# mdejong/MetalHuffman

Hardware: AMD Instinct MI355X
Metric: decoded MB/s (and Mpixels/s) at 2048×1536 grayscale, 1/2/4/8 GPU + CPU ref (higher is better)
Workload: dtype u8; 1 GPU; config2: one 2048x1536 BigBridge-derived frame per launch per GPU; width=2048, height=1536, parallelism=frame-sharded x1

## Files before the change

### metalhuffman_amd/csrc/mh_decode.hip

```cpp
#include <hip/hip_runtime.h>
#include <hip/hip_ext.h>

#include <stdint.h>

#include <atomic>
#include <mutex>

#include "../../include/metalhuffman.h"
#include "mh_lut.hpp"

namespace {

#ifndef MH_DIAG_STAMPS
#define MH_DIAG_STAMPS 0
#endif
#ifndef MH_DIAG_CLOCK
#define MH_DIAG_CLOCK 0
#endif
#ifndef MH_DIAG_ARGS
#define MH_DIAG_ARGS 0
#endif
#ifndef MH_DIAG_DROP_STORES
#define MH_DIAG_DROP_STORES 0
#endif
#ifndef MH_LANE_PAIRS
#define MH_LANE_PAIRS 0
#endif
constexpr int kStageBytes = 4352;
constexpr int kMaxWavesPerWG = 8;
constexpr int kMinWavesPerEU = 6;
constexpr int kBatchStoreAux = 2;
constexpr int kSmallStoreAux = 18;
static_assert(kStageBytes % 16 == 0, "stage uses 16-byte chunks");

typedef unsigned int v4u32 __attribute__((ext_vector_type(4)));

struct DecodeArgs {
  const uint32_t *offsets;
  const uint8_t *codes;
  const uint64_t *frame_off;
  uint64_t codes_bytes;
  const uint16_t *t1;
  const uint16_t *t2;
  const uint16_t *lut;
  const uint8_t *block_init;
  uint8_t *out;
  uint64_t out_pitch;
  uint64_t out_frame_stride;
  uint64_t out_frame_bytes;
  uint32_t t2_entries;
  uint32_t w, h, bw, bh, nb;
  uint32_t tiles_per_frame, total_tiles;
  uint32_t n_groups;
  uint32_t nwaves, grid;
};

__device__ __forceinline__ uint32_t bswap32(uint32_t x) {
  return __builtin_amdgcn_perm(0u, x, 0x00010203u);
}

__device__ __forceinline__ uint32_t split_lookup(const uint16_t *t1, const uint16_t *t2,
                                                 uint32_t t2_entries, uint32_t pat16) {
  uint32_t e = t1[pat16 >> 8];
  if ((e >> 8) == 0) {
    const uint32_t idx = (e & 0xFFu) * 256u + (pat16 & 0xFFu);
    e = idx < t2_entries ? (uint32_t)t2[idx] : 0u;
  }
  return e;
}


template <class SyncFn>
__device__ void build_lut(const uint16_t *t1, const uint16_t *t2, uint32_t t2_entries,
                          uint16_t *lut, uint32_t *p0, uint32_t tid, uint32_t nthreads,
                          SyncFn sync) {
  if (tid == 0) *p0 = (uint32_t)kL1Entries;
  sync();
  for (uint32_t p = tid; p < (uint32_t)kL1Entries; p += nthreads) {
    const uint32_t e = split_lookup(t1, t2, t2_entries, p << kL2Bits);
    lut[p] = (uint16_t)step_word(e);
    if ((e >> 8) > (uint32_t)kLutBits) atomicMin(p0, p);
  }
  for (uint32_t i = tid; i < (uint32_t)(kLutEntries - kL1Entries); i += nthreads)
    lut[kL1Entries + i] = 0;
  sync();
  const uint32_t P0 = *p0;
  for (uint32_t p = P0 + tid; p < (uint32_t)kL1Entries; p += nthreads) {
    const uint32_t sub = p - P0 + 1;
    lut[p] = (uint16_t)(sub < (uint32_t)kL2Subtables ? sub : 0u);
  }
  const uint32_t nl2 = ((uint32_t)kL1Entries - P0) << kL2Bits;
  for (uint32_t i = tid; i < nl2 && i < (uint32_t)(kL2Entries - (1 << kL2Bits)); i += nthreads)
    lut[kL1Entries + (1 << kL2Bits) + i] =
        (uint16_t)step_word(split_lookup(t1, t2, t2_entries, (P0 << kL2Bits) + i));
  sync();
}


#if !MH_LANE_PAIRS
__global__ void __launch_bounds__(1024) mh_prepare_lut_kernel(const uint16_t *t1, const uint16_t *t2,
                                                              uint32_t t2_entries, uint8_t *buf) {
  __shared__ uint16_t s_t1[256];
  __shared__ uint32_t s_scratch[4];
  if (threadIdx.x < 256) s_t1[threadIdx.x] = t1[threadIdx.x];
  __syncthreads();
  build_prepared_lut(s_t1, t2, t2_entries, buf, s_scratch);
}
#endif

struct LdsWords {
  const uint8_t *w;
  __device__ __forceinline__ const uint8_t *at(uint32_t byte_off) const { return w + byte_off; }
};
__device__ __forceinline__ uint32_t swz_off(uint32_t o) { return o ^ ((o >> 3) & 0x70u); }

__device__ __forceinline__ uint32_t pack_prev4(uint32_t a, uint32_t b, uint32_t c, uint32_t d) {
  const uint32_t lo = __builtin_amdgcn_perm(b, a, 0x0C0C0501u);
  const uint32_t hi = __builtin_amdgcn_perm(d, c, 0x05010C0Cu);
  return lo | hi;
}

__device__ __forceinline__ uint32_t pack_lo4(uint32_t a, uint32_t b, uint32_t c, uint32_t d) {
  const uint32_t lo = __builtin_amdgcn_perm(b, a, 0x0C0C0400u);
  const uint32_t hi = __builtin_amdgcn_perm(d, c, 0x04000C0Cu);
  return lo | hi;
}

__device__ __forceinline__ constexpr uint32_t ins_sel1(int j) {
  return j == 0 ? 0x03020105u : j == 1 ? 0x03020500u : j == 2 ? 0x03050100u : 0x05020100u;
}

__shared__ __attribute__((aligned(16))) uint16_t s_lut[kLutEntries];
__shared__ __attribute__((aligned(16))) uint8_t s_stage[kMaxWavesPerWG * kStageBytes];
__shared__ uint32_t s_p0;

#if MH_DIAG_STAMPS
constexpr int kDiagWaves = 8192, kDiagSlots = 8;
__device__ unsigned long long g_stamps[kDiagWaves * kDiagSlots];
#define MH_STAMP(i) (ts[i] = __builtin_amdgcn_s_memrealtime())
#else
#define MH_STAMP(i) ((void)0)
#endif

__device__ __forceinline__ void set_prio(uint32_t p) {
  switch (__builtin_amdgcn_readfirstlane(p) & 3u) {
    case 0: __builtin_amdgcn_s_setprio(0); break;
    case 1: __builtin_amdgcn_s_setprio(1); break;
    case 2: __builtin_amdgcn_s_setprio(2); break;
    default: __builtin_amdgcn_s_setprio(3); break;
  }
}

template <int kBits, bool kMaskedRefill, bool kEscapes = kBits == kLutBits, bool kSwizzle = false,
          int kStoreAux = kBatchStoreAux, bool kLazyRefill = false, bool kFlat8Bytes = false>
struct StepCfg {
  static constexpr bool kLazy = kLazyRefill;
  static constexpr bool kFlat8 = kFlat8Bytes;
  static constexpr int kAux = kStoreAux;
  static constexpr bool kEsc = kEscapes;
  static constexpr bool kSwz = kSwizzle;
  static constexpr bool kMasked = kMaskedRefill;
  static constexpr uint32_t kCur = 127u - (uint32_t)kBits;
  static constexpr uint32_t kMask = (2u << kBits) - 2u;
  static constexpr uint32_t kRefillAt = kCur - 32u;
};

using Lut13 = StepCfg<kLutBits, true>;
using Lut13NoEsc = StepCfg<kLutBits, true, false>;
using Lut13Flat = StepCfg<kLutBits, true, false, true>;

template <bool kDelta, class Cfg, class Src>
__device__ __forceinline__ void decode_block(const Src &src, const uint8_t *lut, uint32_t p,
                                             uint32_t prev, __amdgpu_buffer_rsrc_t out,
                                             uint32_t row0, uint32_t pitch, bool dead) {
  if constexpr (Cfg::kFlat8) {
    typedef const __attribute__((address_space(3))) uint32_t *lds_u32;
    typedef unsigned int v2u32 __attribute__((ext_vector_type(2)));
    const lds_u32 wp = (lds_u32)(src.w + (p >> 5) * 4u);
    const uint32_t sh = p & 31u;
    uint32_t w[17];
#pragma unroll
    for (int j = 0; j < 17; ++j) w[j] = wp[j];
    const uint32_t rbase = dead ? 0x80000000u : row0;
    uint32_t s = prev;
#pragma unroll
    for (uint32_t r = 0; r < 8; ++r) {
      uint32_t c[2];
#pragma unroll
      for (int h = 0; h < 2; ++h) {
        const uint32_t j = 2 * r + h;
        c[h] = (uint32_t)(((((uint64_t)w[j]) << 32 | w[j + 1]) << sh) >> 32);
      }
      v2u32 v;
      if (kDelta) {
        uint32_t sv[4];
#pragma unroll
        for (int h = 0; h < 2; ++h) {
#pragma unroll
          for (int i = 0; i < 4; ++i) sv[i] = s = s + ((c[h] >> (24 - 8 * i)) & 0xFFu);
          const uint32_t o = pack_lo4(sv[0], sv[1], sv[2], sv[3]);
          if (h) v.y = o; else v.x = o;
        }
      } else {
        v.x = bswap32(c[0]);
        v.y = bswap32(c[1]);
      }
      __builtin_amdgcn_raw_buffer_store_b64(v, out, (int)(rbase + r * pitch), 0, Cfg::kAux);
    }
    return;
  }
  typedef const __attribute__((address_space(3))) uint8_t *lds_u8;
  typedef const __attribute__((address_space(3))) uint32_t *lds_u32;
  const lds_u8 base = (lds_u8)src.w;
  lds_u8 wa = base + (p >> 5) * 4u;
  const auto rd = [&](lds_u8 q) -> uint32_t {
    if constexpr (Cfg::kSwz)
      return *(lds_u32)(base + swz_off((uint32_t)(q - base)));
    else
      return *(lds_u32)q;
  };
  uint32_t S = (prev << 8) + Cfg::kCur - (p & 31u);
  uint32_t kRefill = Cfg::kRefillAt;
  if constexpr ((Cfg::kRefillAt & 1u) != 0u) asm("s_mov_b32 %0, %1" : "=s"(kRefill) : "n"(Cfg::kRefillAt));
  uint32_t hi = rd(wa);
  uint32_t lo = rd(wa + 4);
  uint32_t nw = rd(wa + 8);

#define MH_LOOKUP(A1)                                                               \
  uint32_t e = *reinterpret_cast<const uint16_t *>(lut + (A1));
#define MH_FINISH(J, OW)                                                            \
  {                                                                                 \
    if constexpr (Cfg::kEsc) {                                                      \
      const bool esc = e < kEscapeBelow;                                            \
      if (__builtin_expect(__ballot(esc) != 0, 0)) {                                \
        const uint64_t x = (((uint64_t)hi) << 32) | lo;                             \
        const uint32_t x3 = (uint32_t)(x >> ((S - 2u) & 63u)) & 7u;                 \
        const uint32_t e2 = *reinterpret_cast<const uint16_t *>(                    \
            lut + 2u * (kL1Entries + ((e & 0xFFu) << kL2Bits) + x3));               \
        e = esc ? e2 : e;                                                           \
      }                                                                             \
    }                                                                               \
    S += e;                                                                         \
    if (kDelta) {                                                                   \
      sv[J] = S;                           \
    } else {                                                                        \
      OW = __builtin_amdgcn_perm(e + 0xFFu, OW, ins_sel1(J));    \
    }                                                                               \
  }
#define MH_STEP(J, OW)                                                              \
  {                                                                                 \
    const uint64_t x = (((uint64_t)hi) << 32) | lo;                                 \
    MH_LOOKUP((uint32_t)(x >> (S & 63u)) & Cfg::kMask)                              \
    MH_FINISH(J, OW)                                                                \
  }
#define MH_REFILL_C(c)                                                              \
  {                                                                                 \
    hi = c ? lo : hi;                                                               \
    lo = c ? nw : lo;                                                               \
    const uint32_t d = c ? 4u : 0u;                                                 \
    wa += d;                                                                        \
      \
      \
    if constexpr (Cfg::kSwz) asm volatile("" : "+v"(wa));                          \
      \
      \
      \
    if constexpr (Cfg::kMasked) asm volatile("" : "+v"(hi), "+v"(lo));             \
    S += d * 8u;                                                                    \
    if constexpr (!Cfg::kMasked) nw = rd(wa + 8);                                   \
  }
#define MH_STEP_L(J, OW)                                                            \
  {                                                                                 \
    const uint64_t x = (((uint64_t)hi) << 32) | lo;                                 \
    MH_LOOKUP((uint32_t)(x >> (S & 63u)) & Cfg::kMask)                              \
                        \
    const bool c = (S & 0xFFu) <= kRefill;                                         \
    hi = c ? lo : hi;                                                               \
    lo = c ? nw : lo;                                                               \
    const uint32_t d = c ? 4u : 0u;                                                 \
    wa += d;                                                                        \
    S += d * 8u;                                                                    \
      \
      \
    asm volatile("" : "+v"(S), "+v"(hi), "+v"(lo));                                \
      \
     \
     \
    if constexpr (((J) & 1) == 0) nw = rd(wa + 8);                                 \
    MH_FINISH(J, OW)                                                                \
  }
#define MH_STEP_R(J, OW)                                                            \
  {                                                                                 \
    const bool c = (S & 0xFFu) <= kRefill;                                         \
    MH_REFILL_C(c)                                                                  \
    MH_STEP(J, OW)                                                                  \
     \
     \
    if constexpr (Cfg::kMasked) {                                                   \
      if (c) nw = rd(wa + 8);                                                       \
    }                                                                               \
  }

  const uint32_t rbase = (dead || MH_DIAG_DROP_STORES) ? 0x80000000u : row0;
#pragma unroll
  for (uint32_t r = 0; r < 8; ++r) {
    uint32_t o0 = 0, o1 = 0;
    uint32_t sv[4];
    (void)sv;
    if constexpr (Cfg::kLazy) {
      MH_STEP_L(0, o0);
      MH_STEP_L(1, o0);
      MH_STEP_L(2, o0);
      MH_STEP_L(3, o0);
      if (kDelta) o0 = pack_prev4(sv[0], sv[1], sv[2], sv[3]);
      MH_STEP_L(0, o1);
      MH_STEP_L(1, o1);
      MH_STEP_L(2, o1);
      MH_STEP_L(3, o1);
      if (kDelta) o1 = pack_prev4(sv[0], sv[1], sv[2], sv[3]);
    } else {
    if (r) {
      MH_STEP_R(0, o0);
    } else {
      MH_STEP(0, o0);
    }
    MH_STEP(1, o0);
    MH_STEP_R(2, o0);
    MH_STEP(3, o0);
    if (kDelta) o0 = pack_prev4(sv[0], sv[1], sv[2], sv[3]);
    MH_STEP_R(0, o1);
    MH_STEP(1, o1);
    MH_STEP_R(2, o1);
    MH_STEP(3, o1);
    if (kDelta) o1 = pack_prev4(sv[0], sv[1], sv[2], sv[3]);
    }
    {
      typedef unsigned int v2u32 __attribute__((ext_vector_type(2)));
      v2u32 v;
      v.x = o0;
      v.y = o1;
      const uint32_t off = rbase + r * pitch;
      __builtin_amdgcn_raw_buffer_store_b64(v, out, (int)off, 0, Cfg::kAux);
    }
  }
#undef MH_STEP
#undef MH_STEP_R
#undef MH_STEP_L
#undef MH_LOOKUP
#undef MH_FINISH
#undef MH_REFILL_C
}

constexpr int kStageChunks = (kStageBytes / 16 + 63) / 64;

__device__ __forceinline__ __amdgpu_buffer_rsrc_t uniform_rsrc(const void *base, uint32_t bytes) {
  const uint64_t p = (uint64_t)base;
  const uint32_t lo = __builtin_amdgcn_readfirstlane((uint32_t)p);
  const uint32_t hi = __builtin_amdgcn_readfirstlane((uint32_t)(p >> 32));
  return __builtin_amdgcn_make_buffer_rsrc((void *)(((uint64_t)hi << 32) | lo), (short)0,
                                           (int)__builtin_amdgcn_readfirstlane(bytes), 0x00020000);
}

__device__ __forceinline__ uint32_t frame_of(const DecodeArgs &a, uint32_t tile) {
  if (a.total_tiles <= a.tiles_per_frame) return 0u;
  return tile / a.tiles_per_frame;
}

struct TileHdr {
  uint32_t tile;
  uint32_t off;
  uint32_t nxt;
  uint32_t fo_lo, fo_hi;
  uint32_t init;
};

__device__ __forceinline__ void hdr_issue(const DecodeArgs &a, uint32_t tile, uint32_t lane,
                                          TileHdr &h) {
  tile = __builtin_amdgcn_readfirstlane(tile);
  const bool live = tile < a.total_tiles;
  const uint32_t f = live ? frame_of(a, tile) : 0u;
  const uint32_t b = (live ? (tile - f * a.tiles_per_frame) * 64u : 0u) + lane;
  h.tile = tile;
  const __amdgpu_buffer_rsrc_t ro = uniform_rsrc(a.offsets + (uint64_t)f * a.nb, live ? a.nb * 4u : 0u);
  h.off = __builtin_amdgcn_raw_buffer_load_b32(ro, (int)(b * 4u), 0, 0);
  h.nxt = __builtin_amdgcn_raw_buffer_load_b32(ro, (int)(b * 4u + 4u), 0, 0);
  typedef unsigned int v2u32 __attribute__((ext_vector_type(2)));
  const __amdgpu_buffer_rsrc_t rf = uniform_rsrc(
      a.frame_off ? (const void *)a.frame_off : (const void *)a.offsets,
      (live && a.frame_off) ? 0x7FFFFFF0u : 0u);
  const v2u32 v = __builtin_amdgcn_raw_buffer_load_b64(rf, (int)((f + (lane & 1u)) * 8u), 0, 0);
  h.fo_lo = v.x;
  h.fo_hi = v.y;
  const __amdgpu_buffer_rsrc_t ri = uniform_rsrc(
      a.block_init ? (const void *)(a.block_init + (uint64_t)f * a.nb) : (const void *)a.offsets,
      (live && a.block_init) ? a.nb : 0u);
  h.init = __builtin_amdgcn_raw_buffer_load_b8(ri, (int)b, 0, 0);
}

struct Tile {
  uint32_t tile, f, b0;
  bool valid;
  uint32_t p;
  uint32_t start;
  uint32_t span;
  uint32_t fb32;
  uint64_t fbeg;
  uint32_t init;
  uint32_t span_end_bits;
};

__device__ __forceinline__ Tile hdr_resolve(const DecodeArgs &a, const TileHdr &h, uint32_t lane) {
  Tile t;
  t.tile = h.tile;
  t.f = frame_of(a, h.tile);
  t.b0 = (h.tile - t.f * a.tiles_per_frame) * 64u;
  const uint32_t b = t.b0 + lane;
  t.valid = b < a.nb;
  uint64_t fbytes = a.codes_bytes;
  t.fbeg = 0;
  if (a.frame_off) {
    const uint64_t lo = ((uint64_t)__builtin_amdgcn_readlane(h.fo_hi, 0) << 32) |
                        __builtin_amdgcn_readlane(h.fo_lo, 0);
    const uint64_t hi = ((uint64_t)__builtin_amdgcn_readlane(h.fo_hi, 1) << 32) |
                        __builtin_amdgcn_readlane(h.fo_lo, 1);
    t.fbeg = lo;
    fbytes = hi - lo;
  }
  t.fb32 = (uint32_t)(fbytes > 0xFFFFFFF0ull ? 0xFFFFFFF0ull : fbytes);
  const uint32_t fbits = t.fb32 > 0x1FFFFFFFu ? 0xFFFFFFFFu : t.fb32 * 8u;
  const uint32_t end_l = (b + 1u < a.nb) ? h.nxt : min(fbits, h.off + 64u * 16u);
  const uint32_t last = min(63u, a.nb - 1u - t.b0);
  const uint32_t sb = __builtin_amdgcn_readfirstlane(h.off);
  const uint32_t eb = __builtin_amdgcn_readlane(end_l, last);
  t.span_end_bits = eb;
  t.start = (sb >> 3) & ~15u;
  uint32_t end = (eb >> 3) + 24u;
  if (end > t.fb32 + 16u) end = t.fb32 + 16u;
  t.span = end > t.start ? ((end - t.start + 15u) & ~15u) : 0xFFFFFFFFu;
  t.p = t.valid ? h.off - t.start * 8u : 0u;
  t.init = h.init & 0xFFu;
  asm volatile("" ::"v"(t.p), "v"(t.init));
  return t;
}

__device__ __forceinline__ __amdgpu_buffer_rsrc_t codes_rsrc(const DecodeArgs &a, const Tile &t) {
  return uniform_rsrc(a.codes + t.fbeg, t.fb32);
}

struct OutTile {
  __amdgpu_buffer_rsrc_t rsrc;
  uint32_t row0;
};
__device__ __forceinline__ OutTile out_tile(const DecodeArgs &a, const Tile &t, uint32_t lane) {
  const uint32_t b = t.b0 + lane;
  const uint32_t bx = b % a.bw, by = b / a.bw;
  const uint32_t by0 = __builtin_amdgcn_readfirstlane(t.b0 / a.bw);
  const uint64_t base = (uint64_t)by0 * 8u * a.out_pitch;
  const uint64_t rem = a.out_frame_bytes > base ? a.out_frame_bytes - base : 0u;
  OutTile o;
  o.rsrc = uniform_rsrc(a.out + (uint64_t)t.f * a.out_frame_stride + base,
                        (uint32_t)(rem < 0x7FFFFFF0ull ? rem : 0x7FFFFFF0ull));
  o.row0 = (by - by0) * 8u * (uint32_t)a.out_pitch + bx * 8u;
  return o;
}

__device__ __forceinline__ void span_issue(const DecodeArgs &a, const Tile &t, uint32_t lane,
                                           v4u32 (&R)[kStageChunks], bool on = true) {
  const __amdgpu_buffer_rsrc_t rc = uniform_rsrc(a.codes + (on ? t.fbeg : 0ull), on ? t.fb32 : 0u);
  const uint32_t span = __builtin_amdgcn_readfirstlane(on ? t.span : 0u);
#pragma unroll
  for (int k = 0; k < kStageChunks; ++k) {
    const uint32_t c = lane + 64u * k;
    const uint32_t off = c * 16u < span ? t.start + c * 16u : 0xFFFFFFF0u;
    R[k] = __builtin_amdgcn_raw_buffer_load_b128(rc, (int)off, 0, 0);
  }
}

template <bool kSwz = false>
__device__ __forceinline__ void span_write(const Tile &t, uint32_t lane, const v4u32 (&R)[kStageChunks],
                                           uint8_t *stage) {
#pragma unroll
  for (int k = 0; k < kStageChunks; ++k) {
    const uint32_t c = lane + 64u * k;
    if (c * 16u < t.span) {
      v4u32 v = R[k];
      v.x = bswap32(v.x);
      v.y = bswap32(v.y);
      v.z = bswap32(v.z);
      v.w = bswap32(v.w);
      *reinterpret_cast<v4u32 *>(stage + (kSwz ? swz_off(c * 16u) : c * 16u)) = v;
    }
  }
}

__device__ __forceinline__ void lds_barrier() {
  __builtin_amdgcn_fence(__ATOMIC_RELEASE, "workgroup", "local");
  __builtin_amdgcn_s_barrier();
  __builtin_amdgcn_fence(__ATOMIC_ACQUIRE, "workgroup", "local");
}

// ... 427 lines not shown
    const uint32_t sym = sc->sorted[pos];
    return len > 16u ? 0u : ((sym << 8) - len) & 0xFFFFu;
  };
  const auto length_of = [&](uint32_t w) -> uint32_t {
    uint32_t len = 1;
#pragma unroll
    for (int i = 0; i < 16; ++i) len += (uint32_t)(w >= E[i]);
    return len;
  };
  const auto pack8 = [](const uint32_t (&x)[8]) -> v4u32 {
    v4u32 o;
    o.x = x[0] | (x[1] << 16);
    o.y = x[2] | (x[3] << 16);
    o.z = x[4] | (x[5] << 16);
    o.w = x[6] | (x[7] << 16);
    return o;
  };
  v4u32 *lutv = reinterpret_cast<v4u32 *>(lut);
  constexpr uint32_t kL1Chunks = (uint32_t)kL1Entries / 8u;
  static_assert(kL1Chunks == 2u * 64u * kMaxWavesPerWG, "two first-level chunks per thread");
#pragma unroll 1
  for (uint32_t c = tid; c < kL1Chunks; c += 64u * kMaxWavesPerWG) {
    const uint32_t w0 = c << 6, len0 = length_of(w0);
    v4u32 o;
    if (len0 <= 10u) {
      const uint32_t e = entry(w0, len0), e2 = e | (e << 16);
      o.x = o.y = o.z = o.w = e2;
    } else if (len0 > 16u && P0 == (uint32_t)kL1Entries) {
      o.x = o.y = o.z = o.w = 0u;
    } else {
      uint32_t x[8];
#pragma unroll
      for (uint32_t j = 0; j < 8; ++j) {
        const uint32_t p = c * 8u + j, sub = p - P0 + 1u;
        const uint32_t w = p << kL2Bits;
        const uint32_t e = entry(w, length_of(w));
        x[j] = p >= P0 ? (sub < (uint32_t)kL2Subtables ? sub : 0u) : e;
      }
      o = pack8(x);
    }
    lutv[c] = o;
  }
  constexpr uint32_t kL2Chunks = (uint32_t)(kLutEntries - kL1Entries) / 8u;
  const uint32_t j2 = 64u * kMaxWavesPerWG - 1u - tid;
  if (j2 < kL2Chunks) {
    const uint32_t nl2 = ((uint32_t)kL1Entries - P0) << kL2Bits;
    v4u32 o;
    o.x = o.y = o.z = o.w = 0u;
    if (j2 >= 1u && j2 < (uint32_t)kL2Subtables && (j2 - 1u) * 8u < nl2) {
      uint32_t x[8];
#pragma unroll
      for (uint32_t i = 0; i < 8; ++i) {
        const uint32_t w = (P0 << kL2Bits) + (j2 - 1u) * 8u + i;
        x[i] = entry(w, length_of(w));
      }
      o = pack8(x);
    }
    lutv[kL1Chunks + j2] = o;
  }
  return hf;
}

template <bool kDelta>
__global__ void __launch_bounds__(64 * kMaxWavesPerWG, kMinWavesPerEU) mh_decode_headers_kernel(
    const uint32_t *p_offsets, const uint64_t *p_frame_off, const uint8_t *p_block_init, const uint8_t *p_headers,
    const int32_t *p_status, int32_t *p_header_status, uint32_t p_nb, uint32_t p_tiles_per_frame, uint32_t p_groups,
    const DecodeArgs a0) {
  const uint32_t lane = threadIdx.x & 63u;
  const uint32_t wave = __builtin_amdgcn_readfirstlane(threadIdx.x >> 6);
  const uint32_t G = p_groups;
  const uint32_t f = blockIdx.x / G, slice = blockIdx.x - f * G;
  DecodeArgs a = a0;
  a.offsets = p_offsets;
  a.frame_off = p_frame_off;
  a.block_init = p_block_init;
  a.lut = nullptr;
  a.nb = p_nb;
  a.tiles_per_frame = p_tiles_per_frame;
  a.total_tiles = (f + 1u) * p_tiles_per_frame;
  constexpr uint32_t nwaves = kMaxWavesPerWG;
  a.nwaves = nwaves;
  a.grid = G;
  const uint32_t gstride = G * nwaves;
  uint8_t *stage = s_stage + wave * kStageBytes;
  const uint8_t *lut = reinterpret_cast<const uint8_t *>(s_lut);
#if MH_DIAG_STAMPS
  unsigned long long ts[kDiagSlots] = {};
#endif
  MH_STAMP(0);

  const uint32_t t0 = min(f * p_tiles_per_frame + slice * nwaves + wave, a.total_tiles);
  TileHdr hc;
  const uint32_t stv = __builtin_amdgcn_raw_buffer_load_b32(
      uniform_rsrc(p_status ? (const void *)(p_status + f) : (const void *)p_offsets, p_status ? 4u : 0u), 0, 0, 0);
  const uint32_t L = __builtin_amdgcn_raw_buffer_load_b8(uniform_rsrc(p_headers + (uint64_t)f * 256u, 256u),
                                                         (int)threadIdx.x, 0, 0) & 0xFFu;
  hdr_issue(a, t0, lane, hc);
  if (__builtin_amdgcn_readfirstlane(stv) != 0u) return;
  const HeaderFacts hf = header_build(L, s_lut, reinterpret_cast<HeaderScratch *>(s_stage), threadIdx.x, true);
  if (p_header_status && slice == 0 && threadIdx.x == 0) p_header_status[f] = hf.status;
  if (hf.status != MH_OK) return;
  lds_barrier();
  if (hf.flat8)
    flat8_loop<kDelta>(a, lane, stage, lut, t0, gstride, hc MH_TS_ARG);
  else if (hf.mx == hf.mn)
    batch_loop<kDelta, Lut13Flat>(a, lane, stage, lut, t0, gstride, hc, true MH_TS_ARG);
  else if (hf.mx <= (uint32_t)kLutBits)
    batch_loop<kDelta, Lut13NoEsc>(a, lane, stage, lut, t0, gstride, hc, true MH_TS_ARG);
  else
    batch_loop<kDelta, Lut13>(a, lane, stage, lut, t0, gstride, hc, true MH_TS_ARG);
}

__global__ void __launch_bounds__(64 * kMaxWavesPerWG) mh_header_luts_kernel(const uint8_t *headers, uint8_t *luts,
                                                                             uint64_t lut_stride, int32_t *status) {
  const uint32_t hdr = blockIdx.x, tid = threadIdx.x;
  const uint32_t L = tid < 256u ? headers[(uint64_t)hdr * 256u + tid] : 0u;
  const HeaderFacts hf = header_build(L, s_lut, reinterpret_cast<HeaderScratch *>(s_stage), tid, false);
  __syncthreads();
  uint8_t *dst = luts + (uint64_t)hdr * lut_stride;
  const v4u32 *src = reinterpret_cast<const v4u32 *>(s_lut);
  v4u32 zero;
  zero.x = zero.y = zero.z = zero.w = 0u;
  for (uint32_t i = tid; i < (uint32_t)kLutBytes / 16u; i += blockDim.x)
    reinterpret_cast<v4u32 *>(dst)[i] = hf.status == MH_OK ? src[i] : zero;
  if (tid < 4)
    reinterpret_cast<uint32_t *>(dst + kMaxLenOff)[tid] = tid == 0 ? hf.mx : tid == 1 ? hf.mn : tid == 2 ? hf.flat8 : 0u;
  if (status && tid == 0) status[hdr] = hf.status;
}
#endif

constexpr int kSmallWaves = 4;
constexpr int kSmallMaxTilesPerCU = 4;
__shared__ __attribute__((aligned(16))) uint16_t s_lut_small[kLut14Entries];
static_assert(kLutBytes <= kLut14Bytes, "the 13-bit table fits the small kernel's LUT space");

template <bool kDelta>
__device__ __forceinline__ void small_decode(const DecodeArgs &a, const Tile &t, uint32_t lane,
                                             const v4u32 (&R)[kStageChunks], bool live, bool staged, bool flat8,
                                             bool l14, uint8_t *stage, const uint8_t *lut, uint32_t gw MH_TS_PARAM) {
  if (!live) return;
#if MH_DIAG_STAMPS && MH_DIAG_ARGS
  asm volatile("" ::"s"(a.out), "s"((uint32_t)a.out_pitch), "s"((uint32_t)a.out_frame_bytes), "s"(a.bw));
  MH_STAMP(5);
#endif
  const OutTile ot = out_tile(a, t, lane);
  const __amdgpu_buffer_rsrc_t out = ot.rsrc;
  const uint32_t row0 = ot.row0;
  using Small14 = StepCfg<kLut14Bits, false, false, false, kSmallStoreAux, true>;
  using Small13 = StepCfg<kLutBits, false, true, false, kSmallStoreAux, true>;
  using SmallFlat8 = StepCfg<kLutBits, false, false, false, kSmallStoreAux, false, true>;
#if MH_DIAG_STAMPS && MH_DIAG_CLOCK
  unsigned long long c3 = 0;
#endif
  if (staged) {
    span_write(t, lane, R, stage);
    wave_sync();
    MH_STAMP(3);
#if MH_DIAG_STAMPS && MH_DIAG_CLOCK
    c3 = __builtin_amdgcn_s_memtime();
#endif
    LdsWords src{stage};
    if (flat8)
      decode_block<kDelta, SmallFlat8>(src, lut, t.p, t.init, out, row0, (uint32_t)a.out_pitch, !t.valid);
    else if (l14)
      decode_block<kDelta, Small14>(src, lut, t.p, t.init, out, row0, (uint32_t)a.out_pitch, !t.valid);
    else
      decode_block<kDelta, Small13>(src, lut, t.p, t.init, out, row0, (uint32_t)a.out_pitch, !t.valid);
  } else if (flat8) {
    decode_halves<kDelta, SmallFlat8>(a, t, lane, lut, stage, out, row0, !t.valid);
  } else if (l14) {
    decode_halves<kDelta, Small14>(a, t, lane, lut, stage, out, row0, !t.valid);
  } else {
    decode_halves<kDelta, Small13>(a, t, lane, lut, stage, out, row0, !t.valid);
  }
#if MH_DIAG_STAMPS
  MH_STAMP(4);
#if MH_DIAG_CLOCK
  ts[5] = staged ? __builtin_amdgcn_s_memtime() - c3 : 0ull;
#elif !MH_DIAG_ARGS
  ts[5] = ts[4];
#endif
  __builtin_amdgcn_s_waitcnt(0);
  MH_STAMP(6);
  const unsigned xcc = __builtin_amdgcn_s_getreg((3 << 11) | 20);
  ts[7] = ((unsigned long long)xcc << 48) | ((unsigned long long)__smid() << 32) | blockIdx.x;
  if (lane == 0 && gw < (uint32_t)kDiagWaves)
    for (int i = 0; i < kDiagSlots; ++i) g_stamps[gw * kDiagSlots + i] = ts[i];
#else
  (void)gw;
#endif
}

template <bool kDelta>
__global__ void __launch_bounds__(64 * kSmallWaves) mh_decode_small_kernel(
    const uint32_t *p_offsets, const uint64_t *p_frame_off, const uint8_t *p_block_init, const uint16_t *p_lut,
    uint32_t p_nb, uint32_t p_tiles_per_frame, uint32_t p_total_tiles, const DecodeArgs a0) {
  DecodeArgs a = a0;
  a.offsets = p_offsets;
  a.frame_off = p_frame_off;
  a.block_init = p_block_init;
  a.lut = p_lut;
  a.nb = p_nb;
  a.tiles_per_frame = p_tiles_per_frame;
  a.total_tiles = p_total_tiles;
  const uint32_t lane = threadIdx.x & 63u;
  const uint32_t wave = __builtin_amdgcn_readfirstlane(threadIdx.x >> 6);
  constexpr uint32_t nwaves = kSmallWaves;
  uint8_t *stage = s_stage + wave * kStageBytes;
  const uint8_t *lut = reinterpret_cast<const uint8_t *>(s_lut_small);
  const uint8_t *prepared = reinterpret_cast<const uint8_t *>(a.lut);
#if MH_DIAG_STAMPS
  unsigned long long ts[kDiagSlots] = {};
#endif
  MH_STAMP(0);

  const v4u32 lens = *reinterpret_cast<const v4u32 *>(prepared + kMaxLenOff);
  const uint32_t max_len = lens.x;
  const uint32_t tile = min(blockIdx.x * nwaves + wave, a.total_tiles);
  TileHdr h;
  hdr_issue(a, tile, lane, h);
  const bool l14 = max_len <= (uint32_t)kLut14Bits;
  constexpr int kLutLoads = kLut14Bytes / 16 / (64 * kSmallWaves);
  static_assert(kLut14Bytes == kLutLoads * 16 * 64 * kSmallWaves, "whole table per pass");
  v4u32 L[kLutLoads];
  {
    const __amdgpu_buffer_rsrc_t rl =
        uniform_rsrc(prepared + (l14 ? kLut14Off : 0), l14 ? (uint32_t)kLut14Bytes : (uint32_t)kLutBytes);
#pragma unroll
    for (int k = 0; k < kLutLoads; ++k)
      L[k] = __builtin_amdgcn_raw_buffer_load_b128(rl, (int)((threadIdx.x + 64u * kSmallWaves * k) * 16u), 0, 0);
  }
  const Tile t = hdr_resolve(a, h, lane);
  MH_STAMP(1);
  const bool live = t.tile < a.total_tiles;
  const bool staged = live && t.span <= (uint32_t)kStageBytes;
  v4u32 R[kStageChunks];
  span_issue(a, t, lane, R, staged);
  {
    v4u32 *dst = reinterpret_cast<v4u32 *>(s_lut_small);
#pragma unroll
    for (int k = 0; k < kLutLoads; ++k) dst[threadIdx.x + 64u * kSmallWaves * k] = L[k];
  }
  lds_barrier();
  MH_STAMP(2);
  small_decode<kDelta>(a, t, lane, R, live, staged, lens.z != 0u, l14, stage, lut,
                       blockIdx.x * nwaves + wave MH_TS_ARG);
}

constexpr uint32_t kFrameBwShift = 16;
static_assert(MH_MAX_DIM <= 0xFFFFu && (MH_MAX_DIM + 7) / 8 < (1u << (32 - kFrameBwShift)),
              "bw and h share one dword");
template <bool kDelta>
__global__ void __launch_bounds__(64 * kSmallWaves) mh_decode_frame_kernel(
    const uint32_t *p_offsets, const uint16_t *p_lut, const uint8_t *p_codes, uint8_t *p_out,
    const uint8_t *p_block_init, uint32_t p_nb, uint32_t p_codes_bytes, uint32_t p_pitch, uint32_t p_bw_h) {
  DecodeArgs a{};
  a.offsets = p_offsets;
  a.lut = p_lut;
  a.codes = p_codes;
  a.out = p_out;
  a.block_init = p_block_init;
  a.nb = p_nb;
  a.codes_bytes = p_codes_bytes;
  a.out_pitch = p_pitch;
  a.bw = p_bw_h >> kFrameBwShift;
  a.h = p_bw_h & ((1u << kFrameBwShift) - 1u);
  a.out_frame_bytes = (uint64_t)a.h * p_pitch;
  a.tiles_per_frame = a.total_tiles = (p_nb + 63u) / 64u;
  const uint32_t lane = threadIdx.x & 63u;
  const uint32_t wave = __builtin_amdgcn_readfirstlane(threadIdx.x >> 6);
  constexpr uint32_t nwaves = kSmallWaves;
  uint8_t *stage = s_stage + wave * kStageBytes;
  const uint8_t *lut = reinterpret_cast<const uint8_t *>(s_lut_small);
  const uint8_t *prepared = reinterpret_cast<const uint8_t *>(a.lut);
#if MH_DIAG_STAMPS
  unsigned long long ts[kDiagSlots] = {};
#endif
  MH_STAMP(0);

  const uint32_t *lens = reinterpret_cast<const uint32_t *>(prepared + kMaxLenOff);
  const uint32_t max_len = lens[0], flat8 = lens[2];
  const uint32_t tile = min(blockIdx.x * nwaves + wave, a.total_tiles);
  TileHdr h;
  hdr_issue(a, tile, lane, h);
  constexpr int kLutLoads = kLut14Bytes / 16 / (64 * kSmallWaves);
  static_assert(kLut14Bytes == kLutLoads * 16 * 64 * kSmallWaves, "whole table per pass");
  v4u32 L[kLutLoads];
  {
    const __amdgpu_buffer_rsrc_t rl = uniform_rsrc(prepared + kLut14Off, (uint32_t)kLut14Bytes);
#pragma unroll
    for (int k = 0; k < kLutLoads; ++k)
      L[k] = __builtin_amdgcn_raw_buffer_load_b128(rl, (int)((threadIdx.x + 64u * kSmallWaves * k) * 16u), 0, 0);
  }
  const Tile t = hdr_resolve(a, h, lane);
  MH_STAMP(1);
  const bool live = t.tile < a.total_tiles;
  const bool staged = live && t.span <= (uint32_t)kStageBytes;
  v4u32 R[kStageChunks];
  span_issue(a, t, lane, R, staged);
  v4u32 *dst = reinterpret_cast<v4u32 *>(s_lut_small);
#pragma unroll
  for (int k = 0; k < kLutLoads; ++k) dst[threadIdx.x + 64u * kSmallWaves * k] = L[k];
  __builtin_amdgcn_sched_barrier(0);
  const bool l14 = max_len <= (uint32_t)kLut14Bits;
  if (__builtin_expect(!l14, 0)) {
    constexpr uint32_t kChunks = kLutBytes / 16;
    const __amdgpu_buffer_rsrc_t rl = uniform_rsrc(prepared, (uint32_t)kLutBytes);
#pragma unroll 1
    for (uint32_t c = threadIdx.x; c < kChunks; c += 64u * kSmallWaves)
      dst[c] = __builtin_amdgcn_raw_buffer_load_b128(rl, (int)(c * 16u), 0, 0);
  }
  lds_barrier();
  MH_STAMP(2);
  small_decode<kDelta>(a, t, lane, R, live, staged, flat8 != 0u, l14, stage, lut,
                       blockIdx.x * nwaves + wave MH_TS_ARG);
}

#if MH_LANE_PAIRS
constexpr uint32_t kLpMinBits = 16;
constexpr int kLpWaves = 4;
constexpr int kLpStageBytes = 4144;
static_assert(kLpStageBytes <= kStageChunks * 64 * 16, "span_issue covers the lane-pair stage");
constexpr int kLpOutStride = 68;
__shared__ __attribute__((aligned(16))) uint16_t s_lp_lut[kLut14Entries];
__shared__ __attribute__((aligned(16))) uint8_t s_lp_stage[kLpWaves * kLpStageBytes];
__shared__ __attribute__((aligned(16))) uint8_t s_lp_out[kLpWaves * 64 * kLpOutStride];

__device__ __forceinline__ uint32_t lane_xchg(uint32_t lane, uint32_t v) {
  return (uint32_t)__builtin_amdgcn_ds_bpermute((int)((lane ^ 32u) << 2), (int)v);
}

__device__ __forceinline__ uint32_t add_bytes(uint32_t b, uint32_t c) {
  const uint32_t c4 = c * 0x01010101u;
  return ((b & 0x7F7F7F7Fu) + (c4 & 0x7F7F7F7Fu)) ^ ((b ^ c4) & 0x80808080u);
}

template <bool kDelta, class Cfg>
__device__ __forceinline__ void lp_decode(const uint8_t *stage, const uint8_t *lut, uint32_t *row_a,
                                          uint32_t *row_b, uint32_t lane, bool valid, uint32_t p,
                                          uint32_t mid, uint32_t end, bool spec, uint32_t init,
                                          __amdgpu_buffer_rsrc_t out, uint32_t row0, uint32_t pitch) {
  typedef const __attribute__((address_space(3))) uint8_t *lds_u8;
  typedef const __attribute__((address_space(3))) uint32_t *lds_u32;
// ... 311 lines not shown
      hipExtLaunchKernelGGL(kernel, grid, block, 0, s, nullptr, nullptr, hipExtAnyOrderLaunch, __VA_ARGS__); \
    else                                                                                          \
      hipLaunchKernelGGL(kernel, grid, block, 0, s, __VA_ARGS__);                                 \
  } while (0)

template <bool kDelta>
int launch(const DecodeArgs &a0, hipStream_t s, bool lane_pairs, bool any_order) {
  DecodeArgs a = a0;
  const DeviceInfo *di = device_info(s);
  if (!di) return MH_ERR_HIP;
  const int cus = di->cus.load(std::memory_order_relaxed);
#if MH_LANE_PAIRS
  if (lane_pairs && a.lut && a.total_tiles <= (uint32_t)(kSmallMaxTilesPerCU * cus)) {
    const uint32_t n_frames = a.total_tiles / a.tiles_per_frame;
    a.tiles_per_frame = (a.nb + 31u) / 32u;
    a.total_tiles = a.tiles_per_frame * n_frames;
    a.n_groups = (a.total_tiles + kLpWaves - 1) / kLpWaves;
    MH_LAUNCH(mh_decode_lanepair_kernel<kDelta>, dim3(a.n_groups), dim3(kLpWaves * 64), s, any_order, a);
    return hipGetLastError() == hipSuccess ? MH_OK : MH_ERR_HIP;
  }
#else
  (void)lane_pairs;
#endif
  if (a.lut && a.total_tiles <= (uint32_t)(kSmallMaxTilesPerCU * cus)) {
    const uint32_t nw = kSmallWaves;
    a.n_groups = (a.total_tiles + nw - 1) / nw;
    if (a.total_tiles == a.tiles_per_frame && !a.frame_off) {
      MH_LAUNCH(mh_decode_frame_kernel<kDelta>, dim3(a.n_groups), dim3(nw * 64), s, any_order, a.offsets, a.lut,
                a.codes, a.out, a.block_init, a.nb, (uint32_t)a.codes_bytes, (uint32_t)a.out_pitch,
                (a.bw << kFrameBwShift) | a.h);
      return hipGetLastError() == hipSuccess ? MH_OK : MH_ERR_HIP;
    }
    MH_LAUNCH(mh_decode_small_kernel<kDelta>, dim3(a.n_groups), dim3(nw * 64), s, any_order, a.offsets,
              a.frame_off, a.block_init, a.lut, a.nb, a.tiles_per_frame, a.total_tiles, a);
    return hipGetLastError() == hipSuccess ? MH_OK : MH_ERR_HIP;
  }
  uint32_t nw = (a.total_tiles + (uint32_t)cus - 1) / (uint32_t)cus;
  if (nw < 1) nw = 1;
  if (nw > (uint32_t)kMaxWavesPerWG) nw = kMaxWavesPerWG;
  a.n_groups = (a.total_tiles + nw - 1) / nw;
  const uint32_t resident = (uint32_t)(cus * di->occ[kDelta ? 1 : 0][nw]);
  const uint32_t grid = a.n_groups < resident ? a.n_groups : resident;
  a.nwaves = nw;
  a.grid = grid;
  MH_LAUNCH(mh_decode_kernel<kDelta>, dim3(grid), dim3(nw * 64), s, any_order, a.offsets, a.frame_off,
            a.block_init, a.lut, a.nb, a.tiles_per_frame, a.total_tiles, a.nwaves, a.grid, a);
  return hipGetLastError() == hipSuccess ? MH_OK : MH_ERR_HIP;
}

int check_decode_args(const mh_frame *fr, const uint8_t *d_out, size_t out_pitch, size_t out_frame_stride,
                      uint32_t allowed_flags, bool luts, const uint16_t *d_luts, uint64_t lut_stride) {
  if (!fr || !d_out || !fr->d_block_offsets || !fr->d_codes) return MH_ERR_INVALID_ARG;
  if (luts ? !d_luts : (!fr->d_table1 || !fr->d_table2)) return MH_ERR_INVALID_ARG;
  if (fr->n_frames == 0 || (fr->n_frames > 1 && !fr->d_frame_code_offsets)) return MH_ERR_INVALID_ARG;
  if (fr->flags & ~allowed_flags) return MH_ERR_INVALID_ARG;
  const mh_dims &d = fr->dims;
  if (!d.width || !d.height || d.width > MH_MAX_DIM || d.height > MH_MAX_DIM ||
      d.block_width != (d.width + 7) / 8 || d.block_height != (d.height + 7) / 8)
    return MH_ERR_DIMS;
  if (!luts && (fr->table2_entries < 256 || (fr->table2_entries % 256) != 0 ||
                fr->table2_entries > MH_TABLE2_MAX_ENTRIES))
    return MH_ERR_TABLE;
  if (((uintptr_t)fr->d_codes & 15u) || (out_pitch & 7u) || ((uintptr_t)d_out & 7u) ||
      (fr->n_frames > 1 && (out_frame_stride & 7u)))
    return MH_ERR_ALIGN;
  if (luts ? (((uintptr_t)d_luts & 15u) || (lut_stride & 15u)) : (((uintptr_t)fr->d_lut & 15u) != 0))
    return MH_ERR_ALIGN;
  if (out_pitch < d.width || out_pitch > (1u << 20) ||
      (fr->n_frames > 1 && out_frame_stride < out_pitch * d.height))
    return MH_ERR_CAPACITY;
  if (fr->codes_bytes < MH_CODES_PAD) return MH_ERR_CAPACITY;
  if (fr->n_frames == 1 && !fr->d_frame_code_offsets && fr->codes_bytes > 0xFFFFFFF0ull)
    return MH_ERR_CAPACITY;
  if (luts && lut_stride < (uint64_t)kPreparedBytes) return MH_ERR_CAPACITY;
  return MH_OK;
}

int fill_decode_args(const mh_frame *fr, uint8_t *d_out, size_t out_pitch, size_t out_frame_stride,
                     DecodeArgs &a) {
  const mh_dims &d = fr->dims;
  a.offsets = fr->d_block_offsets;
  a.codes = fr->d_codes;
  a.frame_off = fr->d_frame_code_offsets;
  a.codes_bytes = fr->codes_bytes;
  a.block_init = fr->d_block_init;
  a.out = d_out;
  a.out_pitch = out_pitch;
  a.out_frame_stride = out_frame_stride;
  a.out_frame_bytes = (uint64_t)d.height * out_pitch;
  a.w = d.width;
  a.h = d.height;
  a.bw = d.block_width;
  a.bh = d.block_height;
  a.nb = d.block_width * d.block_height;
  a.tiles_per_frame = (a.nb + 63) / 64;
  const uint64_t total = (uint64_t)a.tiles_per_frame * fr->n_frames;
  if (total > 0x7FFFFFFFull) return MH_ERR_CAPACITY;
  a.total_tiles = (uint32_t)total;
  return MH_OK;
}

#if !MH_LANE_PAIRS
int frames_shape(uint32_t n_frames, uint32_t tiles_per_frame, bool delta, hipStream_t s, uint32_t *groups,
                 bool headers = false) {
  const DeviceInfo *di = device_info(s);
  if (!di) return MH_ERR_HIP;
  const int occ = (headers ? di->occ_headers : di->occ_frames)[delta ? 1 : 0];
  const uint64_t resident = (uint64_t)di->cus.load(std::memory_order_relaxed) * (uint64_t)occ;
  const uint64_t want = (resident + n_frames - 1) / n_frames;
  const uint64_t most = (tiles_per_frame + (uint32_t)kMaxWavesPerWG - 1) / (uint32_t)kMaxWavesPerWG;
  *groups = (uint32_t)(want < 1 ? 1 : want > most ? most : want);
  return MH_OK;
}

template <bool kDelta>
int launch_frames(const DecodeArgs &a, uint32_t n_frames, const uint8_t *luts, uint64_t lut_stride,
                  const int32_t *status, hipStream_t s, bool any_order) {
  uint32_t G = 0;
  const int rc = frames_shape(n_frames, a.tiles_per_frame, kDelta, s, &G);
  if (rc != MH_OK) return rc;
  const uint64_t grid = (uint64_t)G * n_frames;
  if (grid > 0x7FFFFFFFull) return MH_ERR_CAPACITY;
  MH_LAUNCH(mh_decode_multitable_kernel<kDelta>, dim3((uint32_t)grid), dim3(kMaxWavesPerWG * 64), s, any_order,
            a.offsets, a.frame_off, a.block_init, luts, status, lut_stride, a.nb, a.tiles_per_frame, G, a);
  return hipGetLastError() == hipSuccess ? MH_OK : MH_ERR_HIP;
}

template <bool kDelta>
int launch_headers(const DecodeArgs &a, uint32_t n_frames, const uint8_t *headers, const int32_t *status,
                   int32_t *header_status, hipStream_t s, bool any_order) {
  uint32_t G = 0;
  const int rc = frames_shape(n_frames, a.tiles_per_frame, kDelta, s, &G, true);
  if (rc != MH_OK) return rc;
  const uint64_t grid = (uint64_t)G * n_frames;
  if (grid > 0x7FFFFFFFull) return MH_ERR_CAPACITY;
  MH_LAUNCH(mh_decode_headers_kernel<kDelta>, dim3((uint32_t)grid), dim3(kMaxWavesPerWG * 64), s, any_order,
            a.offsets, a.frame_off, a.block_init, headers, status, header_status, a.nb, a.tiles_per_frame, G, a);
  return hipGetLastError() == hipSuccess ? MH_OK : MH_ERR_HIP;
}
#endif

}

extern "C" {

#if !MH_LANE_PAIRS

#if MH_DIAG_STAMPS
int mh_diag_stamps(unsigned long long *host, size_t n) {
  if (n > sizeof(g_stamps) / sizeof(g_stamps[0])) n = sizeof(g_stamps) / sizeof(g_stamps[0]);
  return hipMemcpyFromSymbol(host, HIP_SYMBOL(g_stamps), n * sizeof(unsigned long long), 0,
                             hipMemcpyDeviceToHost) == hipSuccess ? (int)n : -1;
}
#endif

#ifdef MH_TABLE_STAMPS
size_t mh_lut_bytes(void) { return (size_t)kPreparedBytes + 256; }
#else
size_t mh_lut_bytes(void) { return (size_t)kPreparedBytes; }
#endif
int mh_lut_bits(void) { return kLutBits; }

int mh_device_count(void) {
  int n = 0;
  if (hipGetDeviceCount(&n) != hipSuccess) return 0;
  return n;
}

int mh_prepare_lut(const mh_lookup_symbol *d_table1, const mh_lookup_symbol *d_table2,
                   uint32_t table2_entries, uint16_t *d_lut, void *stream) {
  if (!d_table1 || !d_table2 || !d_lut) return MH_ERR_INVALID_ARG;
  if (table2_entries < 256 || (table2_entries % 256) != 0 || table2_entries > MH_TABLE2_MAX_ENTRIES)
    return MH_ERR_TABLE;
  if ((uintptr_t)d_lut & 15u) return MH_ERR_ALIGN;
  hipLaunchKernelGGL(mh_prepare_lut_kernel, dim3(1), dim3(1024), 0, (hipStream_t)stream,
                     reinterpret_cast<const uint16_t *>(d_table1),
                     reinterpret_cast<const uint16_t *>(d_table2), table2_entries,
                     reinterpret_cast<uint8_t *>(d_lut));
  return hipGetLastError() == hipSuccess ? MH_OK : MH_ERR_HIP;
}

#endif

#if MH_LANE_PAIRS
int mh_diag_decode_lanepairs(const mh_frame *fr, uint8_t *d_out, size_t out_pitch, size_t out_frame_stride,
                             void *stream) {
#else
int mh_decode(const mh_frame *fr, uint8_t *d_out, size_t out_pitch, size_t out_frame_stride,
              void *stream) {
#endif
  int rc = check_decode_args(fr, d_out, out_pitch, out_frame_stride,
                             MH_FLAG_NO_DELTA | MH_FLAG_ANY_ORDER | MH_FLAG_LANE_PAIRS, false, nullptr, 0);
  if (rc != MH_OK) return rc;
  DecodeArgs a{};
  a.t1 = reinterpret_cast<const uint16_t *>(fr->d_table1);
  a.t2 = reinterpret_cast<const uint16_t *>(fr->d_table2);
  a.lut = fr->d_lut;
  a.t2_entries = fr->table2_entries;
  rc = fill_decode_args(fr, d_out, out_pitch, out_frame_stride, a);
  if (rc != MH_OK) return rc;
  hipStream_t s = (hipStream_t)stream;
  const bool lp = (fr->flags & MH_FLAG_LANE_PAIRS) != 0;
  const bool ao = (fr->flags & MH_FLAG_ANY_ORDER) != 0;
  return (fr->flags & MH_FLAG_NO_DELTA) ? launch<false>(a, s, lp, ao) : launch<true>(a, s, lp, ao);
}

#if !MH_LANE_PAIRS
int mh_decode_frames(const mh_frame *fr, const uint16_t *d_luts, uint64_t lut_stride_bytes,
                     const int32_t *d_frame_status, uint8_t *d_out, size_t out_pitch, size_t out_frame_stride,
                     void *stream) {
  int rc = check_decode_args(fr, d_out, out_pitch, out_frame_stride, MH_FLAG_NO_DELTA | MH_FLAG_ANY_ORDER, true,
                             d_luts, lut_stride_bytes);
  if (rc != MH_OK) return rc;
  DecodeArgs a{};
  rc = fill_decode_args(fr, d_out, out_pitch, out_frame_stride, a);
  if (rc != MH_OK) return rc;
  hipStream_t s = (hipStream_t)stream;
  const uint8_t *luts = reinterpret_cast<const uint8_t *>(d_luts);
  const bool ao = (fr->flags & MH_FLAG_ANY_ORDER) != 0;
  return (fr->flags & MH_FLAG_NO_DELTA)
             ? launch_frames<false>(a, fr->n_frames, luts, lut_stride_bytes, d_frame_status, s, ao)
             : launch_frames<true>(a, fr->n_frames, luts, lut_stride_bytes, d_frame_status, s, ao);
}

int mh_decode_frames_shape(const mh_frame *fr, void *stream, uint32_t *groups_per_frame,
                           uint32_t *waves_per_group) {
  if (!fr || !groups_per_frame || !waves_per_group || fr->n_frames == 0) return MH_ERR_INVALID_ARG;
  if (fr->flags & ~(MH_FLAG_NO_DELTA | MH_FLAG_ANY_ORDER)) return MH_ERR_INVALID_ARG;
  const mh_dims &d = fr->dims;
  if (!d.width || !d.height || d.width > MH_MAX_DIM || d.height > MH_MAX_DIM ||
      d.block_width != (d.width + 7) / 8 || d.block_height != (d.height + 7) / 8)
    return MH_ERR_DIMS;
  const uint32_t tiles = (d.block_width * d.block_height + 63) / 64;
  const int rc = frames_shape(fr->n_frames, tiles, !(fr->flags & MH_FLAG_NO_DELTA), (hipStream_t)stream,
                              groups_per_frame);
  if (rc != MH_OK) return rc;
  *waves_per_group = kMaxWavesPerWG;
  return MH_OK;
}

int mh_decode_headers(const mh_frame *fr, const uint8_t *d_canon_headers, const int32_t *d_frame_status,
                      int32_t *d_header_status, uint8_t *d_out, size_t out_pitch, size_t out_frame_stride,
                      void *stream) {
  if (d_header_status && d_header_status == d_frame_status) return MH_ERR_INVALID_ARG;
  int rc = check_decode_args(fr, d_out, out_pitch, out_frame_stride, MH_FLAG_NO_DELTA | MH_FLAG_ANY_ORDER, true,
                             d_canon_headers ? reinterpret_cast<const uint16_t *>(uintptr_t{16}) : nullptr,
                             (uint64_t)kPreparedBytes);
  if (rc != MH_OK) return rc;
  DecodeArgs a{};
  rc = fill_decode_args(fr, d_out, out_pitch, out_frame_stride, a);
  if (rc != MH_OK) return rc;
  hipStream_t s = (hipStream_t)stream;
  const bool ao = (fr->flags & MH_FLAG_ANY_ORDER) != 0;
  return (fr->flags & MH_FLAG_NO_DELTA)
             ? launch_headers<false>(a, fr->n_frames, d_canon_headers, d_frame_status, d_header_status, s, ao)
             : launch_headers<true>(a, fr->n_frames, d_canon_headers, d_frame_status, d_header_status, s, ao);
}

int mh_decode_headers_shape(const mh_frame *fr, void *stream, uint32_t *groups_per_frame,
                            uint32_t *waves_per_group) {
  if (!fr || !groups_per_frame || !waves_per_group || fr->n_frames == 0) return MH_ERR_INVALID_ARG;
  if (fr->flags & ~(MH_FLAG_NO_DELTA | MH_FLAG_ANY_ORDER)) return MH_ERR_INVALID_ARG;
  const mh_dims &d = fr->dims;
  if (!d.width || !d.height || d.width > MH_MAX_DIM || d.height > MH_MAX_DIM ||
      d.block_width != (d.width + 7) / 8 || d.block_height != (d.height + 7) / 8)
    return MH_ERR_DIMS;
  const uint32_t tiles = (d.block_width * d.block_height + 63) / 64;
  const int rc = frames_shape(fr->n_frames, tiles, !(fr->flags & MH_FLAG_NO_DELTA), (hipStream_t)stream,
                              groups_per_frame, true);
  if (rc != MH_OK) return rc;
  *waves_per_group = kMaxWavesPerWG;
  return MH_OK;
}

int mh_header_luts_device(const uint8_t *d_canon_headers, uint32_t n_headers, uint16_t *d_luts,
                          uint64_t lut_stride_bytes, int32_t *d_status, void *stream) {
  if (!d_canon_headers || !d_luts || n_headers == 0 || n_headers > 65535u) return MH_ERR_INVALID_ARG;
  if (((uintptr_t)d_luts & 15u) || (lut_stride_bytes & 15u)) return MH_ERR_ALIGN;
  if (lut_stride_bytes < mh_lut_bytes()) return MH_ERR_CAPACITY;
  hipLaunchKernelGGL(mh_header_luts_kernel, dim3(n_headers), dim3(kMaxWavesPerWG * 64), 0, (hipStream_t)stream,
                     d_canon_headers, reinterpret_cast<uint8_t *>(d_luts), lut_stride_bytes, d_status);
  return hipGetLastError() == hipSuccess ? MH_OK : MH_ERR_HIP;
}
#endif

}
```

Measured before the change: 656,200 MB/s.

## Software-pipeline lazy LUT lookups and loop decode rows with partial unroll

The lazy decode path now issues the next symbol's LDS table lookup before finishing the current symbol, so LDS latency overlaps the bit-buffer update. The 8-row loop becomes a rolled outer loop of 4 unrolled rows, with a volatile lookup at the trip boundary, which cuts code size and instruction-cache pressure. Branch hints make the 14-bit staged path the expected one. Row-timestamp diagnostics are added behind a compile flag. The risks are a speculative extra lookup past the last symbol and higher register pressure.

```diff
diff --git a/metalhuffman_amd/csrc/mh_decode.hip b/metalhuffman_amd/csrc/mh_decode.hip
--- a/metalhuffman_amd/csrc/mh_decode.hip
+++ b/metalhuffman_amd/csrc/mh_decode.hip
@@ -23,9 +23,21 @@
 #ifndef MH_DIAG_DROP_STORES
 #define MH_DIAG_DROP_STORES 0
 #endif
+#ifndef MH_DIAG_ROWS
+#define MH_DIAG_ROWS 0
+#endif
+#if MH_DIAG_ROWS && !MH_DIAG_STAMPS
+#error "MH_DIAG_ROWS is a mode of the MH_DIAG_STAMPS build"
+#endif
 #ifndef MH_LANE_PAIRS
 #define MH_LANE_PAIRS 0
 #endif
+#ifndef MH_LAZY_ROWS_PER_ITER
+#define MH_LAZY_ROWS_PER_ITER 4
+#endif
+constexpr int kLazyRowsPerIter = MH_LAZY_ROWS_PER_ITER;
+static_assert(kLazyRowsPerIter == 1 || kLazyRowsPerIter == 2 || kLazyRowsPerIter == 4 || kLazyRowsPerIter == 8,
+              "a block's 8 rows in whole trips");
 constexpr int kStageBytes = 4352;
 constexpr int kMaxWavesPerWG = 8;
 constexpr int kMinWavesPerEU = 6;
@@ -137,6 +149,10 @@
 #if MH_DIAG_STAMPS
 constexpr int kDiagWaves = 8192, kDiagSlots = 8;
 __device__ unsigned long long g_stamps[kDiagWaves * kDiagSlots];
+#if MH_DIAG_ROWS
+constexpr int kDiagRowSlots = 16;
+__device__ uint32_t g_rows[kDiagWaves * kDiagRowSlots];
+#endif
 #define MH_STAMP(i) (ts[i] = __builtin_amdgcn_s_memrealtime())
 #else
 #define MH_STAMP(i) ((void)0)
@@ -169,10 +185,19 @@
 using Lut13NoEsc = StepCfg<kLutBits, true, false>;
 using Lut13Flat = StepCfg<kLutBits, true, false, true>;
 
+#if MH_DIAG_ROWS
+#define MH_ROWS_PARAM , uint32_t *rowv = nullptr
+#define MH_ROW_STAMP(r) \
+  if (rowv) *rowv = (threadIdx.x & 63u) == (r) ? (uint32_t)__builtin_amdgcn_s_memtime() : *rowv
+#else
+#define MH_ROWS_PARAM
+#define MH_ROW_STAMP(r) ((void)0)
+#endif
+
 template <bool kDelta, class Cfg, class Src>
 __device__ __forceinline__ void decode_block(const Src &src, const uint8_t *lut, uint32_t p,
                                              uint32_t prev, __amdgpu_buffer_rsrc_t out,
-                                             uint32_t row0, uint32_t pitch, bool dead) {
+                                             uint32_t row0, uint32_t pitch, bool dead MH_ROWS_PARAM) {
   if constexpr (Cfg::kFlat8) {
     typedef const __attribute__((address_space(3))) uint32_t *lds_u32;
     typedef unsigned int v2u32 __attribute__((ext_vector_type(2)));
@@ -269,10 +294,15 @@
     S += d * 8u;                                                                    \
     if constexpr (!Cfg::kMasked) nw = rd(wa + 8);                                   \
   }
-#define MH_STEP_L(J, OW)                                                            \
+#define MH_ISSUE_L() MH_ISSUE_LQ(const)
+#define MH_ISSUE_LQ(Q)                                                              \
   {                                                                                 \
     const uint64_t x = (((uint64_t)hi) << 32) | lo;                                 \
-    MH_LOOKUP((uint32_t)(x >> (S & 63u)) & Cfg::kMask)                              \
+    eL = *(Q __attribute__((address_space(3))) uint16_t *)((lds_u8)lut + ((uint32_t)(x >> (S & 63u)) & Cfg::kMask)); \
+  }
+#define MH_TAIL_L(J, OW)                                                            \
+  {                                                                                 \
+    uint32_t e = eL;                                                                \
                         \
     const bool c = (S & 0xFFu) <= kRefill;                                         \
     hi = c ? lo : hi;                                                               \
@@ -302,23 +332,58 @@
   }
 
   const uint32_t rbase = (dead || MH_DIAG_DROP_STORES) ? 0x80000000u : row0;
+  typedef unsigned int v2u32 __attribute__((ext_vector_type(2)));
+  const auto store_row = [&](uint32_t o0, uint32_t o1, uint32_t off) {
+    v2u32 v;
+    v.x = o0;
+    v.y = o1;
+    __builtin_amdgcn_raw_buffer_store_b64(v, out, (int)off, 0, Cfg::kAux);
+  };
+  MH_ROW_STAMP(8);
+  if constexpr (Cfg::kLazy) {
+    uint32_t eL;
+    uint32_t off = rbase;
+    MH_ISSUE_L();
+#pragma unroll 1
+    for (uint32_t r = 0; r < 8; r += (uint32_t)kLazyRowsPerIter) {
+#pragma unroll
+      for (uint32_t q = 0; q < (uint32_t)kLazyRowsPerIter; ++q) {
+        uint32_t o0 = 0, o1 = 0;
+        uint32_t sv[4];
+        (void)sv;
+        MH_TAIL_L(0, o0);
+        MH_ISSUE_L();
+        MH_TAIL_L(1, o0);
+        MH_ISSUE_L();
+        MH_TAIL_L(2, o0);
+        MH_ISSUE_L();
+        MH_TAIL_L(3, o0);
+        if (kDelta) o0 = pack_prev4(sv[0], sv[1], sv[2], sv[3]);
+        MH_ISSUE_L();
+        MH_TAIL_L(0, o1);
+        MH_ISSUE_L();
+        MH_TAIL_L(1, o1);
+        MH_ISSUE_L();
+        MH_TAIL_L(2, o1);
+        MH_ISSUE_L();
+        MH_TAIL_L(3, o1);
+        if (kDelta) o1 = pack_prev4(sv[0], sv[1], sv[2], sv[3]);
+        if (q + 1 == (uint32_t)kLazyRowsPerIter && kLazyRowsPerIter < 8) {
+          MH_ISSUE_LQ(const volatile);
+        } else {
+          MH_ISSUE_L();
+        }
+        store_row(o0, o1, off);
+        off += pitch;
+        MH_ROW_STAMP(r + q);
+      }
+    }
+  } else {
 #pragma unroll
   for (uint32_t r = 0; r < 8; ++r) {
     uint32_t o0 = 0, o1 = 0;
     uint32_t sv[4];
     (void)sv;
-    if constexpr (Cfg::kLazy) {
-      MH_STEP_L(0, o0);
-      MH_STEP_L(1, o0);
-      MH_STEP_L(2, o0);
-      MH_STEP_L(3, o0);
-      if (kDelta) o0 = pack_prev4(sv[0], sv[1], sv[2], sv[3]);
-      MH_STEP_L(0, o1);
-      MH_STEP_L(1, o1);
-      MH_STEP_L(2, o1);
-      MH_STEP_L(3, o1);
-      if (kDelta) o1 = pack_prev4(sv[0], sv[1], sv[2], sv[3]);
-    } else {
     if (r) {
       MH_STEP_R(0, o0);
     } else {
@@ -333,19 +398,15 @@
     MH_STEP_R(2, o1);
     MH_STEP(3, o1);
     if (kDelta) o1 = pack_prev4(sv[0], sv[1], sv[2], sv[3]);
-    }
-    {
-      typedef unsigned int v2u32 __attribute__((ext_vector_type(2)));
-      v2u32 v;
-      v.x = o0;
-      v.y = o1;
-      const uint32_t off = rbase + r * pitch;
-      __builtin_amdgcn_raw_buffer_store_b64(v, out, (int)off, 0, Cfg::kAux);
-    }
+    store_row(o0, o1, rbase + r * pitch);
+    MH_ROW_STAMP(r);
+  }
   }
 #undef MH_STEP
 #undef MH_STEP_R
-#undef MH_STEP_L
+#undef MH_ISSUE_L
+#undef MH_ISSUE_LQ
+#undef MH_TAIL_L
 #undef MH_LOOKUP
 #undef MH_FINISH
 #undef MH_REFILL_C
@@ -1079,7 +1140,13 @@
 #if MH_DIAG_STAMPS && MH_DIAG_CLOCK
   unsigned long long c3 = 0;
 #endif
-  if (staged) {
+#if MH_DIAG_ROWS
+  uint32_t rowv = 0;
+#define MH_ROWS_ARG , &rowv
+#else
+#define MH_ROWS_ARG
+#endif
+  if (__builtin_expect(staged, 1)) {
     span_write(t, lane, R, stage);
     wave_sync();
     MH_STAMP(3);
@@ -1087,12 +1154,12 @@
     c3 = __builtin_amdgcn_s_memtime();
 #endif
     LdsWords src{stage};
-    if (flat8)
+    if (__builtin_expect(l14 && !flat8, 1))
+      decode_block<kDelta, Small14>(src, lut, t.p, t.init, out, row0, (uint32_t)a.out_pitch, !t.valid MH_ROWS_ARG);
+    else if (flat8)
       decode_block<kDelta, SmallFlat8>(src, lut, t.p, t.init, out, row0, (uint32_t)a.out_pitch, !t.valid);
-    else if (l14)
-      decode_block<kDelta, Small14>(src, lut, t.p, t.init, out, row0, (uint32_t)a.out_pitch, !t.valid);
     else
-      decode_block<kDelta, Small13>(src, lut, t.p, t.init, out, row0, (uint32_t)a.out_pitch, !t.valid);
+      decode_block<kDelta, Small13>(src, lut, t.p, t.init, out, row0, (uint32_t)a.out_pitch, !t.valid MH_ROWS_ARG);
   } else if (flat8) {
     decode_halves<kDelta, SmallFlat8>(a, t, lane, lut, stage, out, row0, !t.valid);
   } else if (l14) {
@@ -1113,9 +1180,13 @@
   ts[7] = ((unsigned long long)xcc << 48) | ((unsigned long long)__smid() << 32) | blockIdx.x;
   if (lane == 0 && gw < (uint32_t)kDiagWaves)
     for (int i = 0; i < kDiagSlots; ++i) g_stamps[gw * kDiagSlots + i] = ts[i];
+#if MH_DIAG_ROWS
+  if (lane < (uint32_t)kDiagRowSlots && gw < (uint32_t)kDiagWaves) g_rows[gw * kDiagRowSlots + lane] = rowv;
+#endif
 #else
   (void)gw;
 #endif
+#undef MH_ROWS_ARG
 }
 
 template <bool kDelta>
@@ -1733,6 +1804,13 @@
   return hipMemcpyFromSymbol(host, HIP_SYMBOL(g_stamps), n * sizeof(unsigned long long), 0,
                              hipMemcpyDeviceToHost) == hipSuccess ? (int)n : -1;
 }
+#if MH_DIAG_ROWS
+int mh_diag_rows(uint32_t *host, size_t n) {
+  if (n > sizeof(g_rows) / sizeof(g_rows[0])) n = sizeof(g_rows) / sizeof(g_rows[0]);
+  return hipMemcpyFromSymbol(host, HIP_SYMBOL(g_rows), n * sizeof(uint32_t), 0, hipMemcpyDeviceToHost) == hipSuccess
+             ? (int)n : -1;
+}
+#endif
 #endif
 
 #ifdef MH_TABLE_STAMPS
```

After: 667,400 MB/s, median of 6. 1.7% higher.
